# arihantb2/direct_lidar_odometry

Measured on AMD Instinct MI355X. Metric: gicp_iterations_per_sec, higher is better.
Workload: dtype f64

## Files before the change

### direct_lidar_odometry_amd/csrc/ngicp_align.h

```cpp
#pragma once

namespace {

std::mutex& persist_mutex(int device) {
  static std::mutex m[64];
  return m[(unsigned)device % 64u];
}

route::Facts route_facts(const ngicp* h, route::Caller caller, int nblocks = 1) {
  route::Facts f;
  f.caller = caller;
  f.persist = h->persist;
  f.robust = h->robust_kind != NGICP_ROBUST_NONE;
  f.prior = h->prior_set;
  f.iterating = h->p.max_iter > 0;
  f.nblocks = nblocks;
  f.pass_slots = h->pass_slots;
  f.persist_slots = h->persist_slots;
  f.max_passes = max_passes(h->p);
  return f;
}
void refuse_for(const ngicp* h, route::Entry e) {
  const std::string why = route::entry_refusal(e, h->voxel_res > 0.0, h->robust_kind != NGICP_ROBUST_NONE, h->prior_set);
  if (!why.empty()) throw ArgError{NGICP_ERR_ARG, why};
// ... 101 lines not shown
    a.tgt_cell_start = nullptr;
    a.tgt_cell_box = nullptr;
    a.cov_tgt = nullptr;
    a.grid = Grid{};
  }
  for (int i = 0; i < 2; ++i) {
    a.tpt[i] = own_buffers ? h->tpt[i].as<float4>() : nullptr;
    a.mahal[i] = own_buffers ? h->mahal[i].as<double>() : nullptr;
  }
  a.gate_sq = h->p.max_corr_dist * h->p.max_corr_dist;
  {
    float f = (float)a.gate_sq;
    if ((double)f < a.gate_sq) f = std::nextafter(f, std::numeric_limits<float>::infinity());
    a.gate_sq_f = f;
  }
  a.batch_far = own_buffers ? h->batch_far.as<unsigned char>() : nullptr;
  a.st = own_buffers ? h->state.as<LmState>() : nullptr;
  a.partials = own_buffers ? h->partials.as<double>() : nullptr;
  a.mode = 3;
  a.dbg_stamps = nullptr;
  a.dbg_qstats = nullptr;
  a.dbg_span = nullptr;
  a.order_valid = order_flag[h->order_sel];
  a.t_first = nullptr;
  a.fused = 0;
  a.persist = 0;
  a.first_pass = 0;
  a.max_passes = 0;
  a.ticket = ctl ? ctl + 1 : nullptr;
  a.gen = own_buffers ? h->gen_lines.as<int>() : nullptr;
// ... 124 lines not shown
      ++counted;
    }
  }
  s.passes_timed = counted;
}

struct Alignment {
  double t_begin = now_ms(), t_loop = 0.0;
  LmState st;
  float loop_ms = 0.f;
  unsigned long spins = 0;
};

void reset_results(ngicp* h) {
  h->hook_valid = 0;
  h->converged = 0;
  h->nr_iterations = 0;
  std::memcpy(h->final_T, kIdentity16, sizeof(kIdentity16));
}

const LmState& upload_initial_state(ngicp* h, const float guess[16]) {
  LmState& st = h->pin_state[0];
  init_state_from_pose(st, pose_from_colmajor(guess));
  if (h->p.max_iter <= 0) st.hot.done = 1;
  HIP_TRY(hipMemcpyAsync(h->state.p, &st, sizeof(st), hipMemcpyHostToDevice, h->stream));
  return st;
}

void begin_alignment(ngicp* h, Alignment& al, const float guess[16], SolveArgs& sa, unsigned long long*& pass_t_first) {
  al.st = upload_initial_state(h, guess);
// ... 41 lines not shown
  s.n_src = (long long)h->src.dev->n;
  s.n_tgt = rolling_active(h) ? (long long)h->roll.n_vox : (long long)h->tgt.dev->n;
  s.host_wait_spins = (long long)al.spins;
  s.align_ms = now_ms() - al.t_begin;
}

void set_pass_mode(const ngicp* h, PassArgs& a) {
  a.mode = (h->p.optimizer == NGICP_OPT_GAUSS_NEWTON) ? 2 : 3;
  if (h->prev_staged_fraction < 0.0 || h->prev_staged_fraction >= 0.12) a.mode |= 32;
}

void allow_k4_only_passes(const ngicp* h, LoopCtx& c, const route::Facts& f) {
  if (!route::honours_lin_unneeded(route::switches(), h->sw, f)) return;
  c.pa.mode |= 64;
  c.sa.pass_honours_word = 1;
}

bool install_xcd_order(ngicp* h, LoopCtx& c) {
  if (!route::switches().xcd_order) return false;
  const int nb = c.nblocks, per = (nb + 7) / 8;
  std::vector<int> ord((size_t)nb);
  std::vector<int> lists[8];
  for (int g = 0; g < nb; ++g) lists[std::min(7, g / per)].push_back(g);
  size_t taken[8] = {0, 0, 0, 0, 0, 0, 0, 0};
  int b = 0;
  for (int placed = 0; placed < nb; ++b) {
    int x = b % 8;
    if (taken[x] >= lists[x].size()) {
      x = 0;
      for (int y = 1; y < 8; ++y)
// ... 184 lines not shown
  HIP_TRY(hipMemsetAsync(h->gen_lines.p, 0, (size_t)kGenLines * kGenStride * sizeof(int), h->stream));
  hipExtLaunchKernelGGL((k_gicp_persist<2, 3>), dim3((unsigned)std::min(c.nblocks, h->persist_slots)), dim3(256), 0, h->stream, start, stop, 0, pa);
}

void do_align(ngicp* h, const float guess[16], float* aligned, size_t out_stride) {
  refuse_route(h, route::Caller::Align, "ngicp_align");
  Alignment al;
  reset_results(h);
  LoopCtx c;
  prepare_loop(h, c);
  if (!(h->order_src == h->src.dev.get() && h->order_groups == c.sa.nblocks)) HIP_TRY(hipMemsetAsync(h->order_flag.p, 0, 4 * sizeof(int), h->stream));
  route::Facts f = route_facts(h, route::Caller::Align, c.nblocks);
  f.xcd_installed = install_xcd_order(h, c);
  set_pass_mode(h, c.pa);
  allow_k4_only_passes(h, c, f);
  if (const char* dbg = std::getenv("NGICP_DEBUG_MODE")) c.pa.mode |= (std::atoi(dbg) & (8 | 16));
  begin_alignment(h, al, guess, c.sa, c.pa.t_first);
  const DebugDumps dbg = debug_begin(h, c);
  f.dump_stamps = dbg.stamp_path != nullptr;
  f.dump_span = dbg.span_path != nullptr;
  f.dump_qstats = dbg.qstat_path != nullptr;
  f.dump_solve = c.sa.dbg_stamps != nullptr;
  const route::Choice pick = route::choose_route(route::switches(), h->sw, f);
  const long max_p = f.max_passes;
  const bool persist_done = pick.route == route::Route::Persist && align_persistent(h, c, al, max_p);
  switch (persist_done ? route::Route::Persist : pick.fallback) {
    case route::Route::Persist:
      break;
    case route::Route::Head:
      head_begin(h);
      feed_alignment(h, al, max_p + 1, [&](long i, hipEvent_t start, hipEvent_t stop) { launch_head(h, c, i, start, stop); });
// ... 392 lines not shown
```

### direct_lidar_odometry_amd/csrc/ngicp_api.hip

```cpp
#include "../../include/ngicp.h"

#include <hip/hip_runtime.h>
#include <hip/hip_ext.h>

#include <algorithm>
#include <atomic>
#include <chrono>
#include <cmath>
#include <cstdio>
#include <cstdlib>
#include <cstring>
#include <limits>
#include <memory>
#include <mutex>
#include <sched.h>
#include <string>
#include <vector>

#include "ngicp_route.h"
#include "ngicp_pass.h"
#include "ngicp_cloudops.h"
#include "ngicp_filters.h"
#include "ngicp_query.h"
#include "ngicp_range.h"
// ... 1435 lines not shown
    if (rows) std::memcpy(rows, h->trace_host.data(), std::min(n, max_rows) * kTraceCols * sizeof(double));
  });
}

int ngicp_get_stats(ngicp_t* h, ngicp_stats* out) {
  if (!h || !out) return NGICP_ERR_ARG;
  if (h->cov_timing_pending) {
    float ms = 0.f;
    if (hipEventSynchronize(h->ev_cov_b) == hipSuccess && hipEventElapsedTime(&ms, h->ev_cov_a, h->ev_cov_b) == hipSuccess) h->stats.covariance_ms = ms;
    h->cov_timing_pending = false;
  }
  h->stats.device_allocs = g_device_allocs.load(std::memory_order_relaxed);
  *out = h->stats;
  return NGICP_OK;
}
int ngicp_set_host_wait(ngicp_t* h, int mode) {
  if (!h || (mode != 0 && mode != 1)) return NGICP_ERR_ARG;
  h->host_wait = mode;
  return NGICP_OK;
}
int ngicp_set_profiling(ngicp_t* h, int on) {
  return guarded(h, [&] {
    h->profiling = on != 0;
    h->prof_stride = on > 1 ? on : 1;
    if (h->profiling && h->prof_events.empty()) {
      h->prof_events.resize(2 * 1024);
      for (auto& e : h->prof_events) HIP_TRY(hipEventCreate(&e));
    }
  });
}
// ... 755 lines not shown
```

### direct_lidar_odometry_amd/csrc/ngicp_handle.h

```cpp
#pragma once

namespace {

thread_local std::string g_create_error;

struct HipError {
  hipError_t code;
  const char* what;
  const char* file;
  int line;
};

#define HIP_TRY(expr)                                          \
  do {                                                         \
    hipError_t _e = (expr);                                    \
    if (_e != hipSuccess) throw HipError{_e, #expr, __FILE__, __LINE__}; \
  } while (0)

struct ArgError {
  int code;
  std::string msg;
};

double now_ms() {
// ... 247 lines not shown
  CovSet src_covs, tgt_covs;

  DevBuf raw, unsorted, keys, counts, fill, tile_sums, tile_sq, tmp, bbox, occ;
  int pass_slots = 768;
  int persist_slots = 0;
  int queue_slots[2] = {768, 1024};
  int persist = 0;
  int order_sel = 0;
  DevBuf grp_order_alt;
  DevBuf gen_lines;
  DevBuf state_alt;
  DevBuf head_ws;
  unsigned long long* pin_ticks = nullptr;
  double prev_staged_fraction = -1.0;
  DevBuf dbg, dbg_q, dbg_s, dbg_span, grp_order, grp_cost, batch_far;
  const void* order_src = nullptr;
  int order_groups = -1;
  DevBuf tpt[2], mahal[2], partials, state, trace, tfinal, out_xyz, scratch16, queries, knn_idx, knn_d2, sums, ticket;
  DevBuf fit_T, fit_part, fit_out, rad_counts, rad_offsets, rad_keys, rad_long;
  size_t rad_total = 0;
  bool rad_valid = false;
  DevBuf range_ws;
  hipEvent_t ev_q_a = nullptr, ev_q_b = nullptr;
  std::vector<hipEvent_t> prof_events;
  int* h_progress = nullptr;
  LmState* pin_state = nullptr;
  LmHot* pin_final = nullptr;
  DevBuf order_flag, t_first;
  int hook_valid = 0;

// ... 178 lines not shown
```

### direct_lidar_odometry_amd/csrc/ngicp_pass.h

```cpp
#pragma once
#include <type_traits>

#include "../../include/ngicp.h"
#include "ngicp_knn.h"
#include "ngicp_terms.h"
#include "ngicp_lm.h"
#include "ngicp_search.h"
#include "ngicp_solve.h"

namespace ngk {

struct PassArgs {
  const float4* qpts;
  const int2* batches;
  const float* batch_boxes;
  const int* grp_order;
  int* grp_cost;
  int n_batches;
  const double* cov_src;
  int n_src;
  const float4* tgt;
  const float4* tgtp;
  const Xyz* tgt3;
  const int* tgt_cell_start;
// ... 15 lines not shown
  const int* order_valid;
  unsigned long long* t_first;
  int fused;
  int* ticket;
  const double* crow_in;
  double* crow_out;
  int* cluster_ticket;
  int* done_flag;
  int persist;
  int first_pass;
  int max_passes;
  int* gen;
  SolveArgs sa;
  int robust_kind;
  double robust_c, robust_c2;
};

constexpr int kStampStride = 24;
#define NG_STAMP(k)                                                                                   \
  do {                                                                                                \
    if (a.dbg_stamps && lane == 0) a.dbg_stamps[(size_t)(blockIdx.x * 4 + wave) * kStampStride + (k)] = __builtin_amdgcn_s_memtime(); \
  } while (0)

template <int G, int WPS = NGICP_PASS_WAVES, bool FUSED = false, bool ROBUST = false>
__global__ void __launch_bounds__(256, WPS) k_gicp_pass(PassArgs a) {
  constexpr int B = 64 / G;
  constexpr int kWin = WPS >= 4 ? 12 : 16, kSideStep = WPS >= 4 ? 8 : 16;
  static_assert(kWin <= kSortedPad, "walk windows may overhang the array by at most the sentinel frame");
  static_assert(B == kBatchQueries, "query batches are built for 32 queries (2 lanes per query)");
  __shared__ double lds[4][kNumSlots];
// ... 158 lines not shown
```

### direct_lidar_odometry_amd/csrc/ngicp_pass_group.inc

```
#ifndef NG_ROBUST
#define NG_ROBUST false
#define NG_ROBUST_DEFAULTED
#endif
  for (int item = group * 4 + wave; item < a.n_batches; item = a.n_batches) {
    typedef const int __attribute__((address_space(4))) * ConstBatchPtr;
    ConstBatchPtr brec = (ConstBatchPtr)(unsigned long long)a.batches + 2 * (size_t)item;
    const int2 it = make_int2(brec[0], brec[1]);
    typedef const float __attribute__((address_space(4))) * ConstBoxPtr;
    const unsigned int far_word = (unsigned int)((ConstBatchPtr)(unsigned long long)a.batch_far)[item >> 2];
    const bool far_before = ((far_word >> (8 * (item & 3))) & 0xffu) != 0;
    ConstBoxPtr bbp = (ConstBoxPtr)(unsigned long long)a.batch_boxes + 6 * (size_t)item;
    const float bb_c0 = bbp[0], bb_c1 = bbp[1], bb_c2 = bbp[2], bb_h0 = bbp[3], bb_h1 = bbp[4], bb_h2 = bbp[5];
    const int qbase = it.x, qcount = it.y, batch = item;
    float mybest = 3.4028234664e38f;
    int mypos = -1;
    const int i = qbase + lane;
    const bool mine = lane < qcount;
    NG_STAMP(1);
    const bool have_prev = NG_HAVE_LIN != 0;
    float4 sp = make_float4(0.f, 0.f, 0.f, 0.f);
    int j_old = -1;
    float4 bp_old = make_float4(0.f, 0.f, 0.f, 0.f);
    double k4 = 0.0;
    double Mold[6] = {0, 0, 0, 0, 0, 0};
    if (mine) {
      sp = a.qpts[i];
      if (have_prev) {
        bp_old = tpt_old[i];
        j_old = __float_as_int(bp_old.w);
      }
// ... 87 lines not shown
      float4 bpo;
      bpo.x = __shfl(bp_old.x, grp); bpo.y = __shfl(bp_old.y, grp); bpo.z = __shfl(bp_old.z, grp); bpo.w = 0.f;
      float qx = 0.f, qy = 0.f, qz = 0.f;
      int cx = 0, cy = 0, cz = 0;
      if (qok) {
        const float3 q = transform_point_rowmajor_f(Tf, qpx, qpy, qpz);
        qx = q.x, qy = q.y, qz = q.z;
        cell_coords(g, qx, qy, qz, cx, cy, cz);
      }
      float best = 3.4028234664e38f;
      int pos = -1;
      if (qok && jp >= 0) {
        best = sqdist(qx, qy, qz, bpo);
        pos = jp;
      }
      NG_STAMP(2);
      bool listed = false;
      if (list_rows) {
        {
          wave_lds_sync();
          for (int lev = 0; lev <= grow; ++lev) {
#pragma unroll
            for (int k = 0; k < kStageRowsPerLane; ++k) {
              const bool on = rn[k] > 0 && rho[k] == lev;
              const unsigned long long m = __ballot(on);
              if (on) S.live[nlive + __popcll(m & ((1ull << lane) - 1ull))] = make_int4(ryz[k], rn[k], rs[k], rk[k]);
              nlive += __popcll(m);
            }
          }
          listed = true;
// ... 1 lines not shown
      }
      NG_STAMP(3);
      if (a.dbg_stamps && lane == 0) {
        unsigned long long* d = a.dbg_stamps + (size_t)(blockIdx.x * 4 + wave) * kStampStride;
        d[10] = (unsigned long long)(listed ? grow : 0);
        d[11] = (unsigned long long)nlive;
        d[12] = (unsigned long long)qcount;
        d[13] = (unsigned long long)((b1x - b0x + 1) | ((b1y - b0y + 1) << 8) | ((b1z - b0z + 1) << 16));
      }
      bool went_far = false;
      const bool in_box = qok && listed && cx >= b0x && cx <= b1x && cy >= b0y && cy <= b1y && cz >= b0z && cz <= b1z;
      unsigned int dbg_g1 = 0, dbg_g2 = 0;
      auto pack_key = [](float d, int p) { return ((unsigned long long)__float_as_uint(d) << 32) | (unsigned int)p; };
      if (qok && sub == 0) {
        if (in_box) ++nstaged;
        S.qtab[grp] = make_float4(qx, qy, qz, 0.f);
        S.qkey[grp] = pack_key(best, pos);
      }
      if (lane == 0) S.q_tail = 0, S.q_head = 0;
      if (a.dbg_qstats && lane < 32) S.qstat[lane][0] = S.qstat[lane][1] = S.qstat[lane][2] = 0;
      wave_lds_sync();
      if (qok) {
        const float lim = fminf(best, a.gate_sq_f);
        constexpr int kRowsPerLane = (9 + G - 1) / G;
        struct alignas(4) Bounds4 { int v[4]; };
        Bounds4 bnd[kRowsPerLane], bxs[kRowsPerLane];
        float gap[kRowsPerLane];
        int code[kRowsPerLane];
#pragma unroll
        for (int k = 0; k < kRowsPerLane; ++k) {
          const int order = sub + k * G;
          const int tt = order == 0 ? 4 : (order < 5 ? 2 * order - 1 : (order == 5 ? 0 : (order == 6 ? 2 : (order == 7 ? 6 : 8))));
          const int z = cz + tt / 3 - 1, y = cy + tt % 3 - 1;
          code[k] = -1;
          gap[k] = 0.f;
          bnd[k] = Bounds4{{0, 0, 0, 0}};
          bxs[k] = Bounds4{{0, 0, 0, 0}};
          if (order < 9 && z >= 0 && z < g.nz && y >= 0 && y < g.ny) {
// ... 26 lines not shown
            S.unit_s[slot] = s0;
            S.unit_e[slot] = e0;
            S.unit_g[slot] = gap[k];
          }
          ntail += __popcll(hm);
        }
        if (lane == 0) S.q_tail = ntail, S.q_head = 64 / kWalkLanes;
      }
      wave_lds_sync();
      int li_pre = sub;
      bool pre_far = false;
#if NGICP_PRE_FAR
      if (listed) {
        if (in_box) {
          const float b1 = unexplored_bound_sq(g, qx, qy, qz, cx, cy, cz, 1);
          pre_far = !(best <= b1 || b1 >= a.gate_sq_f);
        }
        if (__any(pre_far)) {
          if (pre_far) {
            const float lim = fminf(best, a.gate_sq_f);
            const float fxb = fminf(fmaxf((qx - (g.ox + (float)b0x * g.h)) / ((float)(b1x + 1 - b0x) * g.h), 0.f), 1.f);
            for (; li_pre < nlive; li_pre += G) {
              const int4 rec = S.live[li_pre];
              const float gp = row_gap_sq(g, rec.x & 0xffff, rec.x >> 16, cy, cz, qy, qz);
              if (gp > lim) continue;
              const int slot = atomicAdd(&S.q_tail, 1);
              if (slot >= kUnitCap) break;
              const int k0 = rec.w & 0xffff, k1 = (int)((unsigned int)rec.w >> 16);
              S.unit_q[slot] = grp | (9 << 5) | (min(max(k0 + (int)(fxb * (float)(k1 - k0)), 0), (1 << 22) - 1) << 9);
              S.unit_s[slot] = rec.z;
              S.unit_e[slot] = rec.z + rec.y;
              S.unit_g[slot] = gp;
            }
          }
          wave_lds_sync();
// ... 12 lines not shown
            return atomicAdd(&S.q_head, 1);
          } else {
            int nu = 0;
            if (ql == 0) nu = atomicAdd(&S.q_head, 1);
            return quad_perm_i<0x00>(nu);
          }
        };
        for (int u = lane / kWalkLanes; u < tail; u = next_unit()) {
          ++popped;
          const int uq = S.unit_q[u], qs = uq & 31, s0 = S.unit_s[u], e0 = S.unit_e[u];
          const float gyz = S.unit_g[u];
          const float4 q = S.qtab[qs];
          const unsigned long long k0 = S.qkey[qs];
          float ub = __uint_as_float((unsigned int)(k0 >> 32));
          int up = (int)(unsigned int)k0;
          if (gyz > fminf(ub, a.gate_sq_f)) continue;
          const unsigned int c_before = ncand;
          const unsigned int steps_before1 = dbg_g1;
          if constexpr (kWalkLanes == 1) scan_global_outward<kWin, kSideStep>(a.tgt3, s0, e0, s0 + (uq >> 9), q.x, q.y, q.z, gyz, a.gate_sq_f, ub, up, ncand, dbg_g1);
          else scan_quad_outward<kWin, kSideStep>(a.tgt3, s0, e0, s0 + (uq >> 9), q.x, q.y, q.z, gyz, a.gate_sq_f, ub, up, ncand, dbg_g1, ql);
          if (ql == 0) {
            if (a.dbg_qstats) atomicAdd(reinterpret_cast<int*>(a.dbg_qstats + a.n_src) + min((int)((dbg_g1 - steps_before1) & 0xffff), 63), 1);
            atomicMin(&S.qkey[qs], pack_key(ub, up));
            if (a.dbg_qstats) {
              atomicAdd(&S.qstat[qs][0], (int)(ncand - c_before));
              atomicAdd(&S.qstat[qs][1], 1);
            }
          }
        }
        NG_STAMP(17);
        if (a.dbg_stamps) {
          unsigned long long* d = a.dbg_stamps + (size_t)(blockIdx.x * 4 + wave) * kStampStride;
          atomicMax(&d[18], (unsigned long long)popped);
          if (lane == 0) d[19] = (unsigned long long)tail;
        }
      }
      wave_lds_sync();
      if (qok) {
        const unsigned long long k1 = S.qkey[grp];
        best = __uint_as_float((unsigned int)(k1 >> 32));
        pos = (int)(unsigned int)k1;
      }
      NG_STAMP(4);
      float bound1 = 0.f;
      if (qok) {
        bound1 = unexplored_bound_sq(g, qx, qy, qz, cx, cy, cz, 1);
        went_far = !(best <= bound1 || bound1 >= a.gate_sq_f);
      }
      const unsigned int dbg_c1 = ncand;
      unsigned int dbg_rows = 0;
      const bool need_far = in_box && went_far;
      if (listed && __any(need_far && (!pre_far || li_pre < nlive))) {
        int li = pre_far ? li_pre : sub;
        bool more = need_far;
        for (;;) {
          if (lane == 0) S.q_tail = 0, S.q_head = 0;
          wave_lds_sync();
          if (more) {
            const float lim = fminf(best, a.gate_sq_f);
            for (; li < nlive; li += G) {
              const int4 rec = S.live[li];
              if (row_gap_sq(g, rec.x & 0xffff, rec.x >> 16, cy, cz, qy, qz) > lim) continue;
              const int slot = atomicAdd(&S.q_tail, 1);
              if (slot >= kUnitCap) break;
              S.unit_q[slot] = grp | (li << 5);
              ++dbg_rows;
            }
            more = li < nlive;
          }
          wave_lds_sync();
          {
            const int tail = min(S.q_tail, kUnitCap);
            const int ql = lane % kWalkLanes;
            for (;;) {
              int u = 0;
              if (ql == 0) u = atomicAdd(&S.q_head, 1);
              if constexpr (kWalkLanes > 1) u = quad_perm_i<0x00>(u);
              if (u >= tail) break;
              const int unit = S.unit_q[u], qs = unit & 31;
              const int4 rec = S.live[unit >> 5];
              const float4 q = S.qtab[qs];
              int ux, uy, uz;
              cell_coords(g, q.x, q.y, q.z, ux, uy, uz);
              const float gyz = row_gap_sq(g, rec.x & 0xffff, rec.x >> 16, uy, uz, q.y, q.z);
              const unsigned long long k0 = S.qkey[qs];
              float ub = __uint_as_float((unsigned int)(k0 >> 32));
              int up = (int)(unsigned int)k0;
              if (gyz > fminf(ub, a.gate_sq_f)) continue;
              const int s0 = rec.z + (rec.w & 0xffff), e0 = rec.z + (int)((unsigned int)rec.w >> 16);
              const float frac3 = fminf(fmaxf((q.x - (g.ox + (float)b0x * g.h)) / ((float)(b1x + 1 - b0x) * g.h), 0.f), 1.f);
              const unsigned int c_before = ncand;
              const unsigned int steps_before2 = dbg_g2;
              if constexpr (kWalkLanes == 1) scan_global_outward<kWin, kSideStep>(a.tgt3, rec.z, rec.z + rec.y, s0 + (int)(frac3 * (float)(e0 - s0)), q.x, q.y, q.z, gyz, a.gate_sq_f, ub, up, ncand, dbg_g2);
              else scan_quad_outward<kWin, kSideStep>(a.tgt3, rec.z, rec.z + rec.y, s0 + (int)(frac3 * (float)(e0 - s0)), q.x, q.y, q.z, gyz, a.gate_sq_f, ub, up, ncand, dbg_g2, ql);
              if (ql == 0) {
                if (a.dbg_qstats) atomicAdd(reinterpret_cast<int*>(a.dbg_qstats + a.n_src) + 64 + min((int)((dbg_g2 - steps_before2) & 0xffff), 63), 1);
                atomicMin(&S.qkey[qs], pack_key(ub, up));
                if (a.dbg_qstats) {
                  atomicAdd(&S.qstat[qs][2], (int)(ncand - c_before));
                  atomicAdd(&S.qstat[qs][1], 1 << 16);
                }
              }
            }
          }
          wave_lds_sync();
          if (in_box) {
            const unsigned long long k1 = S.qkey[grp];
            best = __uint_as_float((unsigned int)(k1 >> 32));
            pos = (int)(unsigned int)k1;
          }
          if (!__any(more)) break;
        }
      }
      NG_STAMP(5);
      if (a.dbg_stamps && qok) {
        unsigned long long* d = a.dbg_stamps + (size_t)(blockIdx.x * 4 + wave) * kStampStride;
        atomicMax(&d[14], ((unsigned long long)(dbg_g2 & 0xffff) << 48) | ((unsigned long long)(dbg_g2 >> 16) << 32) | ((unsigned long long)dbg_rows << 16) | (ncand - dbg_c1));
        atomicMax(&d[15], ((unsigned long long)(dbg_g1 & 0xffff) << 48) | ((unsigned long long)(dbg_g1 >> 16) << 32) | dbg_c1);
      }
      const unsigned int c_before_shells = ncand;
      if (qok) nn_shells<G>(g, a.tgt3, a.tgt_cell_start, qx, qy, qz, cx, cy, cz, a.gate_sq_f, sub, need_far ? grow : 1, best, pos, ncand);
      if (a.dbg_qstats) {
        if (qok) atomicAdd(&S.qstat[grp][2], (int)(ncand - c_before_shells));
        wave_lds_sync();
        if (qok && sub == 0) a.dbg_qstats[qi] = make_int4(S.qstat[grp][0], S.qstat[grp][1], S.qstat[grp][2], (went_far ? 1 : 0) | (in_box ? 2 : 0) | (pos >= 0 ? 4 : 0));
      }
      {
        const bool any_far = __any(went_far);
        if (lane == 0) a.batch_far[batch] = any_far ? 1 : 0;
      }
      NG_STAMP(6);
      const int src_lane = (lane % B) * G;
      mybest = __shfl(best, src_lane);
      mypos = __shfl(pos, src_lane);
    }
    double acc[kNumSums];
#pragma unroll
    for (int v = 0; v < kNumSums; ++v) acc[v] = 0.0;
    if ((a.mode & 16) && mine) {
      tpt_new[i] = make_float4(0.f, 0.f, 0.f, __int_as_float(mypos));
      acc[27] += (double)mybest;
    } else if (mine) {
      const double ax = (double)sp.x, ay = (double)sp.y, az = (double)sp.z;
      const double tax = R[0] * ax + R[1] * ay + R[2] * az + t[0];
      const double tay = R[3] * ax + R[4] * ay + R[5] * az + t[1];
      const double taz = R[6] * ax + R[7] * ay + R[8] * az + t[2];

      acc[28] += k4;
      if (do_lin) {
        const int pos = mypos;
        const bool valid = (pos >= 0) && ((double)mybest < a.gate_sq);
        if (!valid) tpt_new[i] = make_float4(0.f, 0.f, 0.f, __int_as_float(-1));
        if (valid) {
          ++nvalid;
          const double* CB = a.cov_tgt + (size_t)pos * 6;
          const double* CA = a.cov_src + (size_t)__float_as_int(sp.w) * 6;
          const Xyz bp = a.tgt3[pos];
          double ca[6];
#pragma unroll
          for (int e = 0; e < 6; ++e) ca[e] = CA[e];
          tpt_new[i] = make_float4(bp.x, bp.y, bp.z, __int_as_float(pos));
          double rcr[6], M[6];
          rotate_sym(R, ca, rcr);
#pragma unroll
          for (int e = 0; e < 6; ++e) rcr[e] = CB[e] + rcr[e];
          inv3_sym(rcr, M);
          double* Mo = mahal_new + (size_t)i * 6;
// ... 42 lines not shown
  NG_STAMP(8);
  __syncthreads();
  NG_STAMP(9);
  if (threadIdx.x < kNumSlots) {
    const int v = threadIdx.x;
    const double val = ((lds[0][v] + lds[1][v]) + lds[2][v]) + lds[3][v];
    if (FUSED) __hip_atomic_store(a.partials + (size_t)group * kNumSlots + v, val, __ATOMIC_RELAXED, __HIP_MEMORY_SCOPE_AGENT);
    else a.partials[(size_t)group * kNumSlots + v] = val;
  }
  if (a.dbg_span && threadIdx.x == 0) {
    unsigned long long* d = a.dbg_span + (size_t)blockIdx.x * 4;
    d[1] = __builtin_amdgcn_s_memrealtime();
    d[2] = (unsigned long long)__builtin_amdgcn_s_getreg((31 << 11) | 4) | ((unsigned long long)__builtin_amdgcn_s_getreg((31 << 11) | 20) << 32);
    d[3] = (unsigned long long)(unsigned int)group;
  }
  if (a.grp_cost && threadIdx.x == 0) {
    const int cost = (int)min((__builtin_amdgcn_s_memtime() - t_start) >> 4, 0x7fffffffull);
    if (FUSED) __hip_atomic_store(a.grp_cost + group, cost, __ATOMIC_RELAXED, __HIP_MEMORY_SCOPE_AGENT);
    else a.grp_cost[group] = cost;
  }
#ifdef NG_ROBUST_DEFAULTED
#undef NG_ROBUST
#undef NG_ROBUST_DEFAULTED
#endif
```

### direct_lidar_odometry_amd/csrc/ngicp_route.h

```cpp
#pragma once

#include <algorithm>
#include <cstdlib>
#include <string>

#include "../../include/ngicp.h"

namespace route {

constexpr int kMaxPersistPasses = 2048;

using Lookup = const char* (*)(const char*);
inline const char* from_environment(const char* name) { return std::getenv(name); }

struct ProcessSwitches {
  int pass_impl = 0;
  bool fused = false;
  int queue = 0;
  int pass_wps = 0;
  bool xcd_order = false;
  bool persist_coop = true;
  int persist_one = 0;
  long debug_solve_launch = 0;
};
// ... 12 lines not shown
inline const ProcessSwitches& switches() {
  static const ProcessSwitches p = read_process_switches(from_environment);
  return p;
}

struct HandleSwitches {
  int persist = 0;
  int head = 0;
  int full_last_pass = 0;
  int serial_step = 0;
  int cell_boxes = 0;
  double target_occ = 24.0;
  double voxel = 0.0;
  int chunk = 3;
  int stage_grow = 6;
};
inline HandleSwitches read_handle_switches(Lookup env, int stage_max_grow) {
  HandleSwitches w;
  if (const char* s = env("NGICP_PERSIST")) w.persist = std::atoi(s);
  if (const char* s = env("NGICP_HEAD")) w.head = std::atoi(s);
  if (const char* s = env("NGICP_FULL_LAST_PASS")) w.full_last_pass = std::atoi(s);
  if (const char* s = env("NGICP_SERIAL_STEP")) w.serial_step = std::atoi(s) != 0 ? 1 : 0;
  if (const char* s = env("NGICP_CELL_BOXES")) w.cell_boxes = std::atoi(s);
  if (const char* s = env("NGICP_TARGET_OCC")) w.target_occ = std::max(1.0, std::atof(s));
  if (const char* s = env("NGICP_VOXEL")) w.voxel = std::atof(s);
  if (const char* s = env("NGICP_CHUNK")) w.chunk = std::max(1, std::min(64, std::atoi(s)));
  if (const char* s = env("NGICP_STAGE_GROW")) w.stage_grow = std::max(0, std::min(stage_max_grow, std::atoi(s)));
  return w;
}

enum class Route { Default, Staged, Queue, Fused, Persist, PersistOne, Head };
struct RouteRow {
  Route route;
  const char* asked_by;
  bool robust;
  bool prior;
  bool lin_unneeded;
  bool own_solver;
};
constexpr RouteRow kRoutes[] = {
    {Route::Default, "", true, true, true, true},
    {Route::Staged, "NGICP_PASS_IMPL=1", false, true, false, true},
// ... 72 lines not shown
    case Route::Fused: return align && p.fused;
    case Route::Persist: return align && f.persist != 0;
    case Route::Head: return align && w.head != 0;
    case Route::PersistOne: return align && p.persist_one != 0;
    default: return false;
  }
}

inline bool honours_lin_unneeded(const ProcessSwitches& p, const HandleSwitches& w, const Facts& f) {
  if (f.caller == Caller::Hook || w.full_last_pass || p.pass_impl != 0) return false;
  for (const RouteRow& r : kRoutes)
    if (asked(r.route, p, w, f) && !r.lin_unneeded) return false;
  return true;
}

inline std::string refusal(const ProcessSwitches& p, const HandleSwitches& w, const Facts& f, const char* entry) {
  if (f.caller == Caller::Sharded) return {};
  const bool hook = f.caller == Caller::Hook;
  if (f.robust)
    for (const RouteRow& r : kRoutes)
      if (asked(r.route, p, w, f) && !r.robust)
        return std::string(entry) + ": the robust kernel has no instantiation of the pass variant " + r.asked_by + " selects" +
               (hook ? "" : " (unset it, or ngicp_set_robust_kernel(h, NGICP_ROBUST_NONE, 0))");
  if (f.prior)
    for (const RouteRow& r : kRoutes)
      if (asked(r.route, p, w, f) && !r.prior)
        return std::string(entry) + ": the pose prior is not applied by the route " + r.asked_by + " selects (unset it, or ngicp_set_pose_prior(h, NULL, NULL))";
  return {};
}

// ... 30 lines not shown
```

### direct_lidar_odometry_amd/csrc/ngicp_search.h

```cpp
#pragma once
#include "ngicp_grid.h"

namespace ngk {

struct alignas(4) Xyz { float x, y, z; };
__device__ __forceinline__ float sqdist(float qx, float qy, float qz, const Xyz& p) {
  const float dx = qx - p.x, dy = qy - p.y, dz = qz - p.z;
  float r = dx * dx;
  r = r + dy * dy;
  r = r + dz * dz;
  return r;
}

__device__ __forceinline__ float3 transform_point_rowmajor_f(const float* Tf, float x, float y, float z) {
  float3 q;
  q.x = ((Tf[0] * x + Tf[1] * y) + Tf[2] * z) + Tf[3];
  q.y = ((Tf[4] * x + Tf[5] * y) + Tf[6] * z) + Tf[7];
  q.z = ((Tf[8] * x + Tf[9] * y) + Tf[10] * z) + Tf[11];
  return q;
}

__global__ void __launch_bounds__(256) k_pack_pos(const float4* __restrict__ in, int n_padded, int pad, float4* __restrict__ out) {
  const int i = blockIdx.x * blockDim.x + threadIdx.x;
  if (i >= n_padded) return;
  const float4 p = in[i];
  const bool real = i >= pad && i < n_padded - pad;
  out[i] = make_float4(p.x, p.y, p.z, __int_as_float(real ? i - pad : -1));
}

__global__ void __launch_bounds__(256) k_pack_xyz(const float4* __restrict__ in, int n, Xyz* __restrict__ out) {
  const int i = blockIdx.x * blockDim.x + threadIdx.x;
  if (i >= n) return;
  const float4 p = in[i];
  out[i] = Xyz{p.x, p.y, p.z};
// ... 260 lines not shown
```

### direct_lidar_odometry_amd/nano_gicp.py

```python
from __future__ import annotations

import ctypes as C
import enum
import os
import sys

import numpy as np

_HERE = os.path.dirname(os.path.abspath(__file__))
_LIB_PATH = os.environ.get("NGICP_LIB") or os.path.join(_HERE, "libngicp_hip.so")

c_f32p = C.POINTER(C.c_float)
c_f64p = C.POINTER(C.c_double)
c_i32p = C.POINTER(C.c_int)

FLT_MAX = float(np.finfo(np.float32).max)


class RegularizationMethod(enum.IntEnum):
    NONE = 0
    MIN_EIG = 1
    NORMALIZED_MIN_EIG = 2
    PLANE = 3
    FROBENIUS = 4
# ... 32 lines not shown
                ("voxelmap_ms", C.c_double), ("search_passes", C.c_int)]

    def as_dict(self):
        d = {k: getattr(self, k) for k, _ in self._fields_}
        d["grid_dims"] = list(self.grid_dims)
        return d


EXPORTS = [
    "ngicp_create", "ngicp_destroy", "ngicp_last_error", "ngicp_version", "ngicp_set_params", "ngicp_set_tuning",
    "ngicp_set_source", "ngicp_register_source", "ngicp_set_target", "ngicp_clear_source", "ngicp_clear_target",
    "ngicp_share_source_index", "ngicp_swap_source_target", "ngicp_compute_source_covs", "ngicp_compute_target_covs",
    "ngicp_copy_source_covs", "ngicp_clear_source_covs", "ngicp_clear_target_covs", "ngicp_source_covs_size",
    "ngicp_target_covs_size", "ngicp_get_source_covs", "ngicp_get_target_covs", "ngicp_set_source_covs",
    "ngicp_set_target_covs", "ngicp_align", "ngicp_linearize", "ngicp_compute_error", "ngicp_get_correspondences",
    "ngicp_target_knn", "ngicp_get_lm_trace", "ngicp_get_stats", "ngicp_set_profiling", "ngicp_sharded_begin",
    "ngicp_sharded_pass", "ngicp_sharded_step", "ngicp_sharded_finish",
    "ngicp_keyframe_add", "ngicp_keyframe_add_transformed", "ngicp_keyframe_add_transformed_filtered", "ngicp_keyframe_count", "ngicp_keyframe_size", "ngicp_keyframe_clear",
    "ngicp_submap_set", "ngicp_get_target_points", "ngicp_transform_source", "ngicp_transform_cloud", "ngicp_measure_copy_bandwidth",
    "ngicp_preprocess_scan", "ngicp_set_source_preprocessed", "ngicp_map_add", "ngicp_map_voxel_filter", "ngicp_map_size", "ngicp_map_get",
    "ngicp_map_clear", "ngicp_math_selftest", "ngicp_step_selftest", "ngicp_set_host_wait", "ngicp_covs_shard_begin", "ngicp_covs_shard_compute", "ngicp_covs_shard_commit",
    "ngicp_knn_search", "ngicp_radius_search", "ngicp_radius_fetch", "ngicp_fitness_score",
    "ngicp_align_batch", "ngicp_batch_get_lm_trace", "ngicp_fitness_score_batch",
    "ngicp_range_select", "ngicp_range_median",
    "ngicp_set_voxel_resolution", "ngicp_voxelmap_size", "ngicp_voxelmap_get",
    "ngicp_set_voxel_neighbors", "ngicp_get_voxel_neighbors", "ngicp_voxel_correspondences", "ngicp_voxelmap_builds",
    "ngicp_voxel_align_batch",
    "ngicp_set_voxel_submap_merge", "ngicp_get_voxel_submap_merge", "ngicp_voxelmap_merge_stats", "ngicp_keyframe_voxelmap_get",
    "ngicp_set_voxel_rolling", "ngicp_get_voxel_rolling", "ngicp_voxel_rolling_insert", "ngicp_voxel_rolling_evict", "ngicp_voxel_rolling_clear",
    "ngicp_voxel_rolling_get", "ngicp_voxel_rolling_stats",
    "ngicp_voxel_rolling_set", "ngicp_voxel_rolling_insert_voxels", "ngicp_voxel_rolling_insert_map", "ngicp_voxel_rolling_transform",
# ... 85 lines not shown
    L.ngicp_compute_error.argtypes = [vp, c_f64p, c_f64p]
    L.ngicp_get_correspondences.argtypes = [vp, c_i32p, c_f32p]
    L.ngicp_target_knn.argtypes = [vp, c_f32p, C.c_size_t, C.c_size_t, C.c_int, c_i32p, c_f32p]
    L.ngicp_knn_search.argtypes = [vp, C.c_int, c_f32p, C.c_size_t, C.c_size_t, C.c_int, c_i32p, c_f32p]
    L.ngicp_radius_search.argtypes = [vp, C.c_int, c_f32p, C.c_size_t, C.c_size_t, C.c_double, C.POINTER(C.c_size_t), C.POINTER(C.c_size_t)]
    L.ngicp_radius_fetch.argtypes = [vp, c_i32p, c_f32p, C.c_size_t]
    L.ngicp_fitness_score.argtypes = [vp, c_f32p, C.c_double, c_f64p, C.POINTER(C.c_size_t)]
    L.ngicp_range_select.argtypes = [vp, C.c_int, C.c_size_t, c_f32p, C.POINTER(C.c_size_t)]
    L.ngicp_range_median.argtypes = [vp, C.c_int, c_f32p, C.POINTER(C.c_size_t)]
    L.ngicp_get_lm_trace.argtypes = [vp, c_f64p, C.c_size_t, C.POINTER(C.c_size_t)]
    L.ngicp_align_batch.argtypes = [vp, C.c_size_t, c_f32p, c_f32p, c_i32p, c_i32p, c_f64p]
    L.ngicp_voxel_align_batch.argtypes = [vp, C.c_size_t, c_f32p, c_f32p, c_i32p, c_i32p, c_f64p]
    L.ngicp_batch_get_lm_trace.argtypes = [vp, C.c_size_t, c_f64p, C.c_size_t, C.POINTER(C.c_size_t)]
    L.ngicp_fitness_score_batch.argtypes = [vp, C.c_size_t, c_f32p, C.c_double, c_f64p, C.POINTER(C.c_size_t)]
    L.ngicp_get_stats.argtypes = [vp, C.POINTER(Stats)]
    L.ngicp_set_profiling.argtypes = [vp, C.c_int]
    L.ngicp_sharded_begin.argtypes = [vp, c_f32p]
    L.ngicp_sharded_pass.argtypes = [vp, vp, vp]
    L.ngicp_sharded_step.argtypes = [vp, vp, vp, c_i32p]
    L.ngicp_sharded_finish.argtypes = [vp, c_f32p, c_i32p, c_i32p, c_f64p]
    L.ngicp_keyframe_add.argtypes = [vp, vp, c_i32p]
    L.ngicp_keyframe_add_transformed.argtypes = [vp, vp, c_f32p, c_i32p]
    L.ngicp_keyframe_add_transformed_filtered.argtypes = [vp, vp, c_f32p, C.c_float, c_i32p]
    L.ngicp_keyframe_count.argtypes = [vp, C.POINTER(C.c_size_t)]
    L.ngicp_keyframe_size.argtypes = [vp, C.c_int, C.POINTER(C.c_size_t)]
    L.ngicp_keyframe_clear.argtypes = [vp]
    L.ngicp_keyframe_get.argtypes = [vp, C.c_int, c_f32p, C.c_size_t, c_f64p, C.POINTER(C.c_size_t)]
    L.ngicp_keyframe_transform.argtypes = [vp, c_i32p, C.c_size_t, c_f32p, c_i32p]
    L.ngicp_keyframe_transform_kernel_ms.argtypes = [vp, c_f64p]
    L.ngicp_submap_set.argtypes = [vp, c_i32p, C.c_size_t, c_i32p]
# ... 732 lines not shown
            return out
        self._ck(self._L.ngicp_get_lm_trace(self._h, None, 0, C.byref(n)))
        out = np.empty((n.value, 8))
        if n.value:
            self._ck(self._L.ngicp_get_lm_trace(self._h, _p(out, c_f64p), n.value, C.byref(n)))
        return out

    def setProfiling(self, on):
        self._ck(self._L.ngicp_set_profiling(self._h, int(on)))

    def stats(self) -> dict:
        s = Stats()
        self._ck(self._L.ngicp_get_stats(self._h, C.byref(s)))
        return s.as_dict()

    def addKeyframe(self, producer: "NanoGICP") -> int:
        kid = C.c_int(-1)
        self._ck(self._L.ngicp_keyframe_add(self._h, producer._h, C.byref(kid)))
        return kid.value

    def addKeyframeTransformed(self, producer: "NanoGICP", T) -> int:
        kid = C.c_int(-1)
        t = _colmajor16(T, np.float32)
        self._ck(self._L.ngicp_keyframe_add_transformed(self._h, producer._h, _p(t, c_f32p), C.byref(kid)))
        return kid.value

    def addKeyframeTransformedFiltered(self, producer: "NanoGICP", T, leaf: float) -> int:
        t = _colmajor16(T, np.float32); kid = C.c_int(-1)
        self._ck(self._L.ngicp_keyframe_add_transformed_filtered(self._h, producer._h, _p(t, c_f32p), float(leaf), C.byref(kid)))
        return kid.value
# ... 355 lines not shown
```

### include/ngicp.h

```cpp
#ifndef NGICP_H
#define NGICP_H

#include <stddef.h>
#include <stdint.h>

#ifdef __cplusplus
extern "C" {
#endif

typedef struct ngicp ngicp_t;

#define NGICP_OK 0
#define NGICP_ERR_HIP (-1)
#define NGICP_ERR_ARG (-2)
#define NGICP_ERR_STATE (-3)
#define NGICP_ERR_K_TOO_LARGE (-4)

#define NGICP_REG_NONE 0
#define NGICP_REG_MIN_EIG 1
#define NGICP_REG_NORMALIZED_MIN_EIG 2
#define NGICP_REG_PLANE 3
#define NGICP_REG_FROBENIUS 4

#define NGICP_OPT_GAUSS_NEWTON 0
// ... 136 lines not shown
  double upload_ms;
  double voxel_size;
  int grid_dims[3];
  int lanes_per_query;
  int passes_timed;
  long long n_src, n_tgt;
  double staged_fraction;
  double submap_ms;
  long long device_allocs;
  long long host_wait_spins;
  double query_ms;
  double voxelmap_ms;
  int search_passes;
} ngicp_stats;
int ngicp_get_stats(ngicp_t* h, ngicp_stats* out);
int ngicp_set_profiling(ngicp_t* h, int on);

int ngicp_sharded_begin(ngicp_t* h, const float guess_colmajor[16]);
int ngicp_sharded_pass(ngicp_t* h, double* sums32_dev, void* hip_stream_or_null);
int ngicp_sharded_step(ngicp_t* h, const double* sums32_dev, void* hip_stream_or_null, int* done);
int ngicp_sharded_finish(ngicp_t* h, float T_out_colmajor[16], int* converged, int* nr_iterations, double final_hessian_colmajor[36]);
int ngicp_covs_shard_begin(ngicp_t* h, int which, double** covs6_dev, size_t* n_points);
int ngicp_covs_shard_compute(ngicp_t* h, int which, size_t lo, size_t hi, void* hip_stream_or_null);
int ngicp_covs_shard_commit(ngicp_t* h, int which);

int ngicp_keyframe_add(ngicp_t* h, ngicp_t* from, int* id_out);
int ngicp_keyframe_add_transformed(ngicp_t* h, ngicp_t* from, const float T_colmajor[16], int* id_out);
int ngicp_keyframe_add_transformed_filtered(ngicp_t* h, ngicp_t* from, const float T_colmajor[16], float leaf, int* id_out);
int ngicp_keyframe_count(const ngicp_t* h, size_t* n);
int ngicp_keyframe_size(const ngicp_t* h, int id, size_t* n_points);
// ... 82 lines not shown
```

Measured before the change: 20960.

## Skip nearest-neighbour search for points certified outside the correspondence gate

Adds gate certificates. When a point has no correspondence, the pass searches out to an inflated radius (gate plus a margin) and stores a clearance value in its target slot. On the next pass, if the point has moved less than that clearance, it is certified to still be outside the gate and its search is skipped, reusing the old slot. The aim is to remove repeated full-radius neighbour searches for outlier points. The cost is larger searches when a certificate is issued, extra per-group atomics for statistics, and float rounding margins that must stay conservative for correctness.

```diff
diff --git a/direct_lidar_odometry_amd/csrc/ngicp_align.h b/direct_lidar_odometry_amd/csrc/ngicp_align.h
--- a/direct_lidar_odometry_amd/csrc/ngicp_align.h
+++ b/direct_lidar_odometry_amd/csrc/ngicp_align.h
@@ -139,6 +139,10 @@
     if ((double)f < a.gate_sq) f = std::nextafter(f, std::numeric_limits<float>::infinity());
     a.gate_sq_f = f;
   }
+  a.cert_lim_sq_f = a.gate_sq_f;
+  a.cert_gate_f = 0.f;
+  a.cert_slack_f = 0.f;
+  a.grp_cert = nullptr;
   a.batch_far = own_buffers ? h->batch_far.as<unsigned char>() : nullptr;
   a.st = own_buffers ? h->state.as<LmState>() : nullptr;
   a.partials = own_buffers ? h->partials.as<double>() : nullptr;
@@ -293,6 +297,7 @@
 
 void reset_results(ngicp* h) {
   h->hook_valid = 0;
+  h->cert_groups = 0;
   h->converged = 0;
   h->nr_iterations = 0;
   std::memcpy(h->final_T, kIdentity16, sizeof(kIdentity16));
@@ -364,6 +369,21 @@
   if (!route::honours_lin_unneeded(route::switches(), h->sw, f)) return;
   c.pa.mode |= 64;
   c.sa.pass_honours_word = 1;
+}
+
+void allow_gate_certificates(ngicp* h, LoopCtx& c, const route::Facts& f) {
+  h->cert_groups = 0;
+  if (!route::honours_gate_cert(route::switches(), h->sw, f)) return;
+  const double gate = h->p.max_corr_dist, reach = gate + h->sw.gate_cert_margin;
+  const float lim = (float)(reach * reach);
+  if (!(gate > 0.0) || !std::isfinite(lim) || !(lim > c.pa.gate_sq_f)) return;
+  h->grp_cert.ensure((size_t)c.nblocks * 2 * sizeof(int));
+  c.pa.mode |= 256;
+  c.pa.cert_lim_sq_f = lim;
+  c.pa.cert_gate_f = std::nextafter((float)gate, std::numeric_limits<float>::infinity());
+  c.pa.cert_slack_f = (float)(1e-3 + 4e-6 * reach);
+  c.pa.grp_cert = h->grp_cert.as<int>();
+  h->cert_groups = c.nblocks;
 }
 
 bool install_xcd_order(ngicp* h, LoopCtx& c) {
@@ -578,7 +598,8 @@
   f.xcd_installed = install_xcd_order(h, c);
   set_pass_mode(h, c.pa);
   allow_k4_only_passes(h, c, f);
-  if (const char* dbg = std::getenv("NGICP_DEBUG_MODE")) c.pa.mode |= (std::atoi(dbg) & (8 | 16));
+  allow_gate_certificates(h, c, f);
+  if (const char* dbg = std::getenv("NGICP_DEBUG_MODE")) c.pa.mode |= (std::atoi(dbg) & (8 | 16 | 128));
   begin_alignment(h, al, guess, c.sa, c.pa.t_first);
   const DebugDumps dbg = debug_begin(h, c);
   f.dump_stamps = dbg.stamp_path != nullptr;
diff --git a/direct_lidar_odometry_amd/csrc/ngicp_api.hip b/direct_lidar_odometry_amd/csrc/ngicp_api.hip
--- a/direct_lidar_odometry_amd/csrc/ngicp_api.hip
+++ b/direct_lidar_odometry_amd/csrc/ngicp_api.hip
@@ -1473,6 +1473,18 @@
   *out = h->stats;
   return NGICP_OK;
 }
+int ngicp_get_gate_cert_stats(ngicp_t* h, long long* certified_total, long long* inflated_total) {
+  return guarded(h, [&] {
+    if (!certified_total || !inflated_total) throw ArgError{NGICP_ERR_ARG, "null output"};
+    *certified_total = 0;
+    *inflated_total = 0;
+    if (h->cert_groups <= 0) return;
+    std::vector<int> hc((size_t)h->cert_groups * 2);
+    HIP_TRY(hipMemcpyAsync(hc.data(), h->grp_cert.p, hc.size() * sizeof(int), hipMemcpyDeviceToHost, h->stream));
+    HIP_TRY(hipStreamSynchronize(h->stream));
+    for (size_t g = 0; g < hc.size(); g += 2) *certified_total += hc[g], *inflated_total += hc[g + 1];
+  });
+}
 int ngicp_set_host_wait(ngicp_t* h, int mode) {
   if (!h || (mode != 0 && mode != 1)) return NGICP_ERR_ARG;
   h->host_wait = mode;
diff --git a/direct_lidar_odometry_amd/csrc/ngicp_handle.h b/direct_lidar_odometry_amd/csrc/ngicp_handle.h
--- a/direct_lidar_odometry_amd/csrc/ngicp_handle.h
+++ b/direct_lidar_odometry_amd/csrc/ngicp_handle.h
@@ -285,6 +285,8 @@
   unsigned long long* pin_ticks = nullptr;
   double prev_staged_fraction = -1.0;
   DevBuf dbg, dbg_q, dbg_s, dbg_span, grp_order, grp_cost, batch_far;
+  DevBuf grp_cert;
+  int cert_groups = 0;
   const void* order_src = nullptr;
   int order_groups = -1;
   DevBuf tpt[2], mahal[2], partials, state, trace, tfinal, out_xyz, scratch16, queries, knn_idx, knn_d2, sums, ticket;
diff --git a/direct_lidar_odometry_amd/csrc/ngicp_pass.h b/direct_lidar_odometry_amd/csrc/ngicp_pass.h
--- a/direct_lidar_odometry_amd/csrc/ngicp_pass.h
+++ b/direct_lidar_odometry_amd/csrc/ngicp_pass.h
@@ -53,6 +53,10 @@
   SolveArgs sa;
   int robust_kind;
   double robust_c, robust_c2;
+  float cert_lim_sq_f;
+  float cert_gate_f;
+  float cert_slack_f;
+  int* grp_cert;
 };
 
 constexpr int kStampStride = 24;
diff --git a/direct_lidar_odometry_amd/csrc/ngicp_pass_group.inc b/direct_lidar_odometry_amd/csrc/ngicp_pass_group.inc
--- a/direct_lidar_odometry_amd/csrc/ngicp_pass_group.inc
+++ b/direct_lidar_odometry_amd/csrc/ngicp_pass_group.inc
@@ -14,6 +14,7 @@
     const int qbase = it.x, qcount = it.y, batch = item;
     float mybest = 3.4028234664e38f;
     int mypos = -1;
+    float mylim = a.gate_sq_f;
     const int i = qbase + lane;
     const bool mine = lane < qcount;
     NG_STAMP(1);
@@ -131,6 +132,17 @@
         best = sqdist(qx, qy, qz, bpo);
         pos = jp;
       }
+      float qlim = a.gate_sq_f;
+      if (have_prev && (a.mode & (128 | 256))) {
+        if (qok && jp < 0) qlim = ((a.mode & 128) || cert_holds(qx, qy, qz, bpo.x, bpo.y, bpo.z, jp)) ? -1.f : a.cert_lim_sq_f;
+        if (a.grp_cert) {
+          const int n_cert = __popcll(__ballot(qlim < 0.f && sub == 0)), n_infl = __popcll(__ballot(qlim > a.gate_sq_f && sub == 0));
+          if (lane == 0 && (n_cert | n_infl)) {
+            atomicAdd(a.grp_cert + 2 * group, n_cert);
+            atomicAdd(a.grp_cert + 2 * group + 1, n_infl);
+          }
+        }
+      }
       NG_STAMP(2);
       bool listed = false;
       if (list_rows) {
@@ -162,14 +174,14 @@
       auto pack_key = [](float d, int p) { return ((unsigned long long)__float_as_uint(d) << 32) | (unsigned int)p; };
       if (qok && sub == 0) {
         if (in_box) ++nstaged;
-        S.qtab[grp] = make_float4(qx, qy, qz, 0.f);
+        S.qtab[grp] = make_float4(qx, qy, qz, qlim);
         S.qkey[grp] = pack_key(best, pos);
       }
       if (lane == 0) S.q_tail = 0, S.q_head = 0;
       if (a.dbg_qstats && lane < 32) S.qstat[lane][0] = S.qstat[lane][1] = S.qstat[lane][2] = 0;
       wave_lds_sync();
       if (qok) {
-        const float lim = fminf(best, a.gate_sq_f);
+        const float lim = fminf(best, qlim);
         constexpr int kRowsPerLane = (9 + G - 1) / G;
         struct alignas(4) Bounds4 { int v[4]; };
         Bounds4 bnd[kRowsPerLane], bxs[kRowsPerLane];
@@ -226,11 +238,11 @@
       if (listed) {
         if (in_box) {
           const float b1 = unexplored_bound_sq(g, qx, qy, qz, cx, cy, cz, 1);
-          pre_far = !(best <= b1 || b1 >= a.gate_sq_f);
+          pre_far = !(best <= b1 || b1 >= qlim);
         }
         if (__any(pre_far)) {
           if (pre_far) {
-            const float lim = fminf(best, a.gate_sq_f);
+            const float lim = fminf(best, qlim);
             const float fxb = fminf(fmaxf((qx - (g.ox + (float)b0x * g.h)) / ((float)(b1x + 1 - b0x) * g.h), 0.f), 1.f);
             for (; li_pre < nlive; li_pre += G) {
               const int4 rec = S.live[li_pre];
@@ -273,11 +285,11 @@
           const unsigned long long k0 = S.qkey[qs];
           float ub = __uint_as_float((unsigned int)(k0 >> 32));
           int up = (int)(unsigned int)k0;
-          if (gyz > fminf(ub, a.gate_sq_f)) continue;
+          if (gyz > fminf(ub, q.w)) continue;
           const unsigned int c_before = ncand;
           const unsigned int steps_before1 = dbg_g1;
-          if constexpr (kWalkLanes == 1) scan_global_outward<kWin, kSideStep>(a.tgt3, s0, e0, s0 + (uq >> 9), q.x, q.y, q.z, gyz, a.gate_sq_f, ub, up, ncand, dbg_g1);
-          else scan_quad_outward<kWin, kSideStep>(a.tgt3, s0, e0, s0 + (uq >> 9), q.x, q.y, q.z, gyz, a.gate_sq_f, ub, up, ncand, dbg_g1, ql);
+          if constexpr (kWalkLanes == 1) scan_global_outward<kWin, kSideStep>(a.tgt3, s0, e0, s0 + (uq >> 9), q.x, q.y, q.z, gyz, q.w, ub, up, ncand, dbg_g1);
+          else scan_quad_outward<kWin, kSideStep>(a.tgt3, s0, e0, s0 + (uq >> 9), q.x, q.y, q.z, gyz, q.w, ub, up, ncand, dbg_g1, ql);
           if (ql == 0) {
             if (a.dbg_qstats) atomicAdd(reinterpret_cast<int*>(a.dbg_qstats + a.n_src) + min((int)((dbg_g1 - steps_before1) & 0xffff), 63), 1);
             atomicMin(&S.qkey[qs], pack_key(ub, up));
@@ -304,7 +316,7 @@
       float bound1 = 0.f;
       if (qok) {
         bound1 = unexplored_bound_sq(g, qx, qy, qz, cx, cy, cz, 1);
-        went_far = !(best <= bound1 || bound1 >= a.gate_sq_f);
+        went_far = !(best <= bound1 || bound1 >= qlim);
       }
       const unsigned int dbg_c1 = ncand;
       unsigned int dbg_rows = 0;
@@ -316,7 +328,7 @@
           if (lane == 0) S.q_tail = 0, S.q_head = 0;
           wave_lds_sync();
           if (more) {
-            const float lim = fminf(best, a.gate_sq_f);
+            const float lim = fminf(best, qlim);
             for (; li < nlive; li += G) {
               const int4 rec = S.live[li];
               if (row_gap_sq(g, rec.x & 0xffff, rec.x >> 16, cy, cz, qy, qz) > lim) continue;
@@ -345,13 +357,13 @@
               const unsigned long long k0 = S.qkey[qs];
               float ub = __uint_as_float((unsigned int)(k0 >> 32));
               int up = (int)(unsigned int)k0;
-              if (gyz > fminf(ub, a.gate_sq_f)) continue;
+              if (gyz > fminf(ub, q.w)) continue;
               const int s0 = rec.z + (rec.w & 0xffff), e0 = rec.z + (int)((unsigned int)rec.w >> 16);
               const float frac3 = fminf(fmaxf((q.x - (g.ox + (float)b0x * g.h)) / ((float)(b1x + 1 - b0x) * g.h), 0.f), 1.f);
               const unsigned int c_before = ncand;
               const unsigned int steps_before2 = dbg_g2;
-              if constexpr (kWalkLanes == 1) scan_global_outward<kWin, kSideStep>(a.tgt3, rec.z, rec.z + rec.y, s0 + (int)(frac3 * (float)(e0 - s0)), q.x, q.y, q.z, gyz, a.gate_sq_f, ub, up, ncand, dbg_g2);
-              else scan_quad_outward<kWin, kSideStep>(a.tgt3, rec.z, rec.z + rec.y, s0 + (int)(frac3 * (float)(e0 - s0)), q.x, q.y, q.z, gyz, a.gate_sq_f, ub, up, ncand, dbg_g2, ql);
+              if constexpr (kWalkLanes == 1) scan_global_outward<kWin, kSideStep>(a.tgt3, rec.z, rec.z + rec.y, s0 + (int)(frac3 * (float)(e0 - s0)), q.x, q.y, q.z, gyz, q.w, ub, up, ncand, dbg_g2);
+              else scan_quad_outward<kWin, kSideStep>(a.tgt3, rec.z, rec.z + rec.y, s0 + (int)(frac3 * (float)(e0 - s0)), q.x, q.y, q.z, gyz, q.w, ub, up, ncand, dbg_g2, ql);
               if (ql == 0) {
                 if (a.dbg_qstats) atomicAdd(reinterpret_cast<int*>(a.dbg_qstats + a.n_src) + 64 + min((int)((dbg_g2 - steps_before2) & 0xffff), 63), 1);
                 atomicMin(&S.qkey[qs], pack_key(ub, up));
@@ -378,7 +390,7 @@
         atomicMax(&d[15], ((unsigned long long)(dbg_g1 & 0xffff) << 48) | ((unsigned long long)(dbg_g1 >> 16) << 32) | dbg_c1);
       }
       const unsigned int c_before_shells = ncand;
-      if (qok) nn_shells<G>(g, a.tgt3, a.tgt_cell_start, qx, qy, qz, cx, cy, cz, a.gate_sq_f, sub, need_far ? grow : 1, best, pos, ncand);
+      if (qok) nn_shells<G>(g, a.tgt3, a.tgt_cell_start, qx, qy, qz, cx, cy, cz, qlim, sub, need_far ? grow : 1, best, pos, ncand);
       if (a.dbg_qstats) {
         if (qok) atomicAdd(&S.qstat[grp][2], (int)(ncand - c_before_shells));
         wave_lds_sync();
@@ -392,6 +404,7 @@
       const int src_lane = (lane % B) * G;
       mybest = __shfl(best, src_lane);
       mypos = __shfl(pos, src_lane);
+      mylim = __shfl(qlim, src_lane);
     }
     double acc[kNumSums];
 #pragma unroll
@@ -409,7 +422,16 @@
       if (do_lin) {
         const int pos = mypos;
         const bool valid = (pos >= 0) && ((double)mybest < a.gate_sq);
-        if (!valid) tpt_new[i] = make_float4(0.f, 0.f, 0.f, __int_as_float(-1));
+        if (!valid) {
+          float4 slot = make_float4(0.f, 0.f, 0.f, __int_as_float(-1));
+          if (mylim < 0.f) {
+            slot = tpt_old[i];
+          } else if (mylim > a.gate_sq_f) {
+            const float3 q = transform_point_rowmajor_f(Tf, sp.x, sp.y, sp.z);
+            slot = make_float4(q.x, q.y, q.z, __int_as_float(-1 - cert_clearance(fminf(mybest, mylim), a.cert_gate_f, a.cert_slack_f, q.x, q.y, q.z)));
+          }
+          tpt_new[i] = slot;
+        }
         if (valid) {
           ++nvalid;
           const double* CB = a.cov_tgt + (size_t)pos * 6;
@@ -482,6 +504,7 @@
     d[2] = (unsigned long long)__builtin_amdgcn_s_getreg((31 << 11) | 4) | ((unsigned long long)__builtin_amdgcn_s_getreg((31 << 11) | 20) << 32);
     d[3] = (unsigned long long)(unsigned int)group;
   }
+  if (a.grp_cert && !NG_HAVE_LIN && threadIdx.x == 0) a.grp_cert[2 * group] = 0, a.grp_cert[2 * group + 1] = 0;
   if (a.grp_cost && threadIdx.x == 0) {
     const int cost = (int)min((__builtin_amdgcn_s_memtime() - t_start) >> 4, 0x7fffffffull);
     if (FUSED) __hip_atomic_store(a.grp_cost + group, cost, __ATOMIC_RELAXED, __HIP_MEMORY_SCOPE_AGENT);
diff --git a/direct_lidar_odometry_amd/csrc/ngicp_route.h b/direct_lidar_odometry_amd/csrc/ngicp_route.h
--- a/direct_lidar_odometry_amd/csrc/ngicp_route.h
+++ b/direct_lidar_odometry_amd/csrc/ngicp_route.h
@@ -50,6 +50,8 @@
   double voxel = 0.0;
   int chunk = 3;
   int stage_grow = 6;
+  int gate_cert = 1;
+  double gate_cert_margin = 0.10;
 };
 inline HandleSwitches read_handle_switches(Lookup env, int stage_max_grow) {
   HandleSwitches w;
@@ -62,6 +64,8 @@
   if (const char* s = env("NGICP_VOXEL")) w.voxel = std::atof(s);
   if (const char* s = env("NGICP_CHUNK")) w.chunk = std::max(1, std::min(64, std::atoi(s)));
   if (const char* s = env("NGICP_STAGE_GROW")) w.stage_grow = std::max(0, std::min(stage_max_grow, std::atoi(s)));
+  if (const char* s = env("NGICP_GATE_CERT")) w.gate_cert = std::atoi(s) != 0 ? 1 : 0;
+  if (const char* s = env("NGICP_GATE_CERT_MARGIN")) w.gate_cert_margin = std::max(0.0, std::min(10.0, std::atof(s)));
   return w;
 }
 
@@ -164,6 +168,13 @@
   return true;
 }
 
+inline bool honours_gate_cert(const ProcessSwitches& p, const HandleSwitches& w, const Facts& f) {
+  if (!w.gate_cert || f.caller != Caller::Align || p.pass_impl != 0 || p.queue != 0) return false;
+  for (const RouteRow& r : kRoutes)
+    if (r.route != Route::Default && asked(r.route, p, w, f)) return false;
+  return true;
+}
+
 inline std::string refusal(const ProcessSwitches& p, const HandleSwitches& w, const Facts& f, const char* entry) {
   if (f.caller == Caller::Sharded) return {};
   const bool hook = f.caller == Caller::Hook;
diff --git a/direct_lidar_odometry_amd/csrc/ngicp_search.h b/direct_lidar_odometry_amd/csrc/ngicp_search.h
--- a/direct_lidar_odometry_amd/csrc/ngicp_search.h
+++ b/direct_lidar_odometry_amd/csrc/ngicp_search.h
@@ -18,6 +18,20 @@
   q.y = ((Tf[4] * x + Tf[5] * y) + Tf[6] * z) + Tf[7];
   q.z = ((Tf[8] * x + Tf[9] * y) + Tf[10] * z) + Tf[11];
   return q;
+}
+
+constexpr float kCertUnit = 1.f / 4096.f;
+constexpr int kCertMaxUnits = 1 << 20;
+__device__ __forceinline__ int cert_clearance(float limit_sq, float gate_up, float slack0, float px, float py, float pz) {
+  const float D = sqrtf(limit_sq) * (1.f - 1e-6f);
+  const float c = (D - gate_up) - (slack0 + 2e-6f * fmaxf(fmaxf(fabsf(px), fabsf(py)), fabsf(pz)));
+  return c > 0.f ? (int)fminf(c * (1.f / kCertUnit), (float)kCertMaxUnits) : 0;
+}
+__device__ __forceinline__ bool cert_holds(float qx, float qy, float qz, float px, float py, float pz, int w) {
+  const float c = (float)(-1 - w) * kCertUnit;
+  const float dx = qx - px, dy = qy - py, dz = qz - pz;
+  const float e2 = (dx * dx + dy * dy) + dz * dz;
+  return w < -1 && w >= -1 - kCertMaxUnits && e2 * (1.f + 1e-5f) < c * c;
 }
 
 __global__ void __launch_bounds__(256) k_pack_pos(const float4* __restrict__ in, int n_padded, int pad, float4* __restrict__ out) {
diff --git a/direct_lidar_odometry_amd/nano_gicp.py b/direct_lidar_odometry_amd/nano_gicp.py
--- a/direct_lidar_odometry_amd/nano_gicp.py
+++ b/direct_lidar_odometry_amd/nano_gicp.py
@@ -70,7 +70,7 @@
     "ngicp_copy_source_covs", "ngicp_clear_source_covs", "ngicp_clear_target_covs", "ngicp_source_covs_size",
     "ngicp_target_covs_size", "ngicp_get_source_covs", "ngicp_get_target_covs", "ngicp_set_source_covs",
     "ngicp_set_target_covs", "ngicp_align", "ngicp_linearize", "ngicp_compute_error", "ngicp_get_correspondences",
-    "ngicp_target_knn", "ngicp_get_lm_trace", "ngicp_get_stats", "ngicp_set_profiling", "ngicp_sharded_begin",
+    "ngicp_target_knn", "ngicp_get_lm_trace", "ngicp_get_stats", "ngicp_get_gate_cert_stats", "ngicp_set_profiling", "ngicp_sharded_begin",
     "ngicp_sharded_pass", "ngicp_sharded_step", "ngicp_sharded_finish",
     "ngicp_keyframe_add", "ngicp_keyframe_add_transformed", "ngicp_keyframe_add_transformed_filtered", "ngicp_keyframe_count", "ngicp_keyframe_size", "ngicp_keyframe_clear",
     "ngicp_submap_set", "ngicp_get_target_points", "ngicp_transform_source", "ngicp_transform_cloud", "ngicp_measure_copy_bandwidth",
@@ -186,6 +186,7 @@
     L.ngicp_batch_get_lm_trace.argtypes = [vp, C.c_size_t, c_f64p, C.c_size_t, C.POINTER(C.c_size_t)]
     L.ngicp_fitness_score_batch.argtypes = [vp, C.c_size_t, c_f32p, C.c_double, c_f64p, C.POINTER(C.c_size_t)]
     L.ngicp_get_stats.argtypes = [vp, C.POINTER(Stats)]
+    L.ngicp_get_gate_cert_stats.argtypes = [vp, C.POINTER(C.c_longlong), C.POINTER(C.c_longlong)]
     L.ngicp_set_profiling.argtypes = [vp, C.c_int]
     L.ngicp_sharded_begin.argtypes = [vp, c_f32p]
     L.ngicp_sharded_pass.argtypes = [vp, vp, vp]
@@ -948,6 +949,11 @@
         self._ck(self._L.ngicp_get_stats(self._h, C.byref(s)))
         return s.as_dict()
 
+    def gateCertificateStats(self) -> dict:
+        c, i = C.c_longlong(0), C.c_longlong(0)
+        self._ck(self._L.ngicp_get_gate_cert_stats(self._h, C.byref(c), C.byref(i)))
+        return {"gate_certified_total": c.value, "gate_inflated_total": i.value}
+
     def addKeyframe(self, producer: "NanoGICP") -> int:
         kid = C.c_int(-1)
         self._ck(self._L.ngicp_keyframe_add(self._h, producer._h, C.byref(kid)))
diff --git a/include/ngicp.h b/include/ngicp.h
--- a/include/ngicp.h
+++ b/include/ngicp.h
@@ -174,6 +174,7 @@
   int search_passes;
 } ngicp_stats;
 int ngicp_get_stats(ngicp_t* h, ngicp_stats* out);
+int ngicp_get_gate_cert_stats(ngicp_t* h, long long* certified_total, long long* inflated_total);
 int ngicp_set_profiling(ngicp_t* h, int on);
 
 int ngicp_sharded_begin(ngicp_t* h, const float guess_colmajor[16]);
```

Measured after the change: 20440. 0.975x the previous value.
